# ak110/object_detector

Measured on AMD Instinct MI355X. Metric: images_per_sec, higher is better.
Workload: dtype f16

## Files before the change

### object_detector_amd/csrc/common.h

```cpp
#pragma once
#include <hip/hip_runtime.h>
#include <stdarg.h>
#include <stdint.h>
#include <stdio.h>
#include <string.h>

#include <unordered_map>

#include "../../include/odhip.h"

struct od_ctx {
  int device;
  void* zero_page;
  float* ones;
  int num_cu;
  std::unordered_map<const void*, size_t> lds_attr;
};

int od_ensure_lds(od_ctx* ctx, const void* fn, size_t lds);

void od_set_error(const char* fmt, ...);

#define OD_CHECK_HIP(expr)                                                                   \
  do {                                                                                       \
// ... 15 lines not shown

#define OD_REQUIRE(cond, ...)   \
  do {                          \
    if (!(cond)) {              \
      od_set_error(__VA_ARGS__); \
      return OD_ERR_INVALID;    \
    }                           \
  } while (0)

typedef _Float16 f16;
typedef f16 f16x8 __attribute__((ext_vector_type(8)));
typedef f16 f16x4 __attribute__((ext_vector_type(4)));
typedef float f32x4 __attribute__((ext_vector_type(4)));

static inline int od_ceil_div(int a, int b) { return (a + b - 1) / b; }
static inline int od_round_up(int a, int b) { return od_ceil_div(a, b) * b; }

struct od_launch {
  const char* name;
  int (*issue)(const od_launch& l, hipStream_t stream);
  const void* fn;
  dim3 grid, block;
  size_t lds;
  alignas(16) unsigned char args[352];
  template <class T> const T& arg() const { return *reinterpret_cast<const T*>(args); }
};
struct od_launches {
  int n = 0;
  od_launch l[6];
};

template <class T>
int od_add_launch(od_launches* L, od_launch l, const T& args) {
  static_assert(sizeof(T) <= sizeof(l.args) && alignof(T) <= 16, "kernel arguments do not fit an od_launch");
  OD_REQUIRE(L->n < 6, "%s: more than 6 launches in one op", l.name);
  memcpy(l.args, &args, sizeof(T));
  L->l[L->n++] = l;
  return OD_OK;
}
static inline int od_issue(const od_launches& L, hipStream_t stream) {
  for (int i = 0; i < L.n; ++i)
    if (int rc = L.l[i].issue(L.l[i], stream)) return rc;
  return OD_OK;
}

template <class F, class... A>
int od_prepare_issue(void* stream, F prepare, A... args) {
// ... 44 lines not shown
```

### object_detector_amd/csrc/conv_8ph_kernel.h

```cpp
#pragma once
#include "conv_8ph_tile.h"
#include "conv_common.h"

namespace {

constexpr int E_ALO = 0, E_AHI = E_REGION, E_BLO = 2 * E_REGION, E_BHI = 3 * E_REGION;

struct TapWalk {
  int c0, tap, tapoff, dx;
  int sel_tap;
};

constexpr unsigned E_OOB = 0x80000000u;

template <int MT, int NF = 4, bool KEEP = false>
static __device__ __forceinline__ void e8_epilogue_rt(const ConvKP& p, f32x4 (&acc)[MT][NF], int m0w, int n0w, int l15,
                                                          int lq, f16x8 (*keep)[NF / 2] = nullptr, int mrows = MT * 16,
                                                          const float* pre_sc = nullptr, const float* pre_bi = nullptr) {
  unsigned pb[MT], ppix[MT];
#pragma unroll
  for (int i = 0; i < MT; ++i) {
    const int m = m0w + i * 16 + l15;
    pb[i] = (unsigned)m / (unsigned)p.HoWo;
    ppix[i] = (unsigned)m - pb[i] * (unsigned)p.HoWo;
  }
#pragma unroll
  for (int pr = 0; pr < NF / 2; ++pr) {
    const int n = n0w + (2 * pr + (lq & 1)) * 16 + (lq >> 1) * 8;
    const bool nok = n < p.Cout;
    float sc[8], bi[8];
    if (pre_sc) {
#pragma unroll
      for (int e = 0; e < 8; ++e) {
        sc[e] = pre_sc[e];
        bi[e] = pre_bi[e];
      }
    } else {
      const f32x4 s0 = *(const f32x4*)(p.scale + n), s1 = *(const f32x4*)(p.scale + n + 4);
      const f32x4 b0 = *(const f32x4*)(p.bias + n), b1 = *(const f32x4*)(p.bias + n + 4);
#pragma unroll
      for (int e = 0; e < 4; ++e) {
        sc[e] = s0[e];
        sc[4 + e] = s1[e];
        bi[e] = b0[e];
        bi[4 + e] = b1[e];
      }
    }
    f16x8 rv[MT];
#pragma unroll
    for (int i = 0; i < MT; ++i) {
      const int m = m0w + i * 16 + l15;
      f16x8 r = {0, 0, 0, 0, 0, 0, 0, 0};
      if (nok && m < p.M && p.res_mode != OD_RES_NONE) {
        long long roff;
        if (p.res_mode == OD_RES_SAME) {
          roff = (long long)m * p.Cout + n;
        } else {
          const unsigned ho = ppix[i] / (unsigned)p.Wo, wo = ppix[i] - ho * (unsigned)p.Wo;
          roff = ((long long)(pb[i] * (unsigned)(p.Ho >> 1) + (ho >> 1)) * (p.Wo >> 1) + (wo >> 1)) * p.Cout + n;
        }
        r = *(const f16x8*)(p.res + roff);
      }
      rv[i] = r;
    }
#pragma unroll
    for (int i = 0; i < MT; ++i) {
      const int m = m0w + i * 16 + l15;
      const bool ok = nok && m < p.M && i * 16 + l15 < mrows;
      float v[8];
#pragma unroll
      for (int e = 0; e < 4; ++e) {
        float a = acc[i][2 * pr][e], bq = acc[i][2 * pr + 1][e];
        od_permlane16_swap(a, bq);
        v[e] = a;
        v[4 + e] = bq;
      }
#pragma unroll
      for (int e = 0; e < 8; ++e) v[e] = v[e] * sc[e] + bi[e];
      if (p.act == OD_ACT_LEAKY) {
#pragma unroll
        for (int e = 0; e < 8; ++e) v[e] = od_leaky(v[e], p.alpha);
      } else if (p.act == OD_ACT_ELU) {
#pragma unroll
        for (int e = 0; e < 8; ++e) v[e] = v[e] > 0.f ? v[e] : p.alpha * od_expm1_fast(v[e]);
      }
      if (p.res_mode != OD_RES_NONE) {
#pragma unroll
        for (int e = 0; e < 8; ++e) v[e] += (float)rv[i][e];
      }
      if (ok) {
        const long long ooff = (long long)pb[i] * p.obs + (long long)ppix[i] * p.ops + n;
        if (p.out_f32) {
          float* o = (float*)p.out + ooff;
          *(f32x4*)o = f32x4{v[0], v[1], v[2], v[3]};
          *(f32x4*)(o + 4) = f32x4{v[4], v[5], v[6], v[7]};
        } else {
          f16x8 h;
#pragma unroll
          for (int e = 0; e < 8; ++e) h[e] = (f16)v[e];
          *(f16x8*)((f16*)p.out + ooff) = h;
        }
      }
      if (KEEP) {
        f16x8 h;
#pragma unroll
        for (int e = 0; e < 8; ++e) h[e] = (f16)v[e];
        keep[i][pr] = h;
      }
    }
  }
}

template <int EPI, int MT, int NF, bool KEEP>
static __device__ __forceinline__ void e8_epilogue_fixed(const ConvKP& p, f32x4 (&acc)[MT][NF], int m0w, int n0w, int l15, int lq,
                                                         f16x8 (*keep)[NF / 2], int mrows, const float* pre_sc,
                                                         const float* pre_bi) {
  constexpr int ACT = od_epi_act(EPI), RES = od_epi_res(EPI);
  constexpr bool F32 = od_epi_f32(EPI);
  unsigned orow[MT], rrow[RES != OD_RES_NONE ? MT : 1];
#pragma unroll
  for (int i = 0; i < MT; ++i) {
    const unsigned m = (unsigned)min(m0w + i * 16 + l15, p.M - 1);
    const unsigned b = m / (unsigned)p.HoWo, pix = m - b * (unsigned)p.HoWo;
    orow[i] = b * (unsigned)p.obs + pix * (unsigned)p.ops;
    if (RES == OD_RES_SAME) rrow[i] = m * (unsigned)p.Cout;
    if (RES == OD_RES_UP2) {
      const unsigned ho = pix / (unsigned)p.Wo, wo = pix - ho * (unsigned)p.Wo;
      rrow[i] = ((b * (unsigned)(p.Ho >> 1) + (ho >> 1)) * (unsigned)(p.Wo >> 1) + (wo >> 1)) * (unsigned)p.Cout;
    }
  }
#pragma unroll
  for (int pr = 0; pr < NF / 2; ++pr) {
    const int n = n0w + (2 * pr + (lq & 1)) * 16 + (lq >> 1) * 8;
    const bool nok = n < p.Cout;
    float sc[8], bi[8];
    if (pre_sc) {
#pragma unroll
      for (int e = 0; e < 8; ++e) {
        sc[e] = pre_sc[e];
        bi[e] = pre_bi[e];
      }
    } else {
      const f32x4 s0 = *(const f32x4*)(p.scale + n), s1 = *(const f32x4*)(p.scale + n + 4);
      const f32x4 b0 = *(const f32x4*)(p.bias + n), b1 = *(const f32x4*)(p.bias + n + 4);
#pragma unroll
      for (int e = 0; e < 4; ++e) {
        sc[e] = s0[e];
        sc[4 + e] = s1[e];
        bi[e] = b0[e];
        bi[4 + e] = b1[e];
      }
// ... 49 lines not shown
  if constexpr (EPI == OD_EPI_RT)
    e8_epilogue_rt<MT, NF, KEEP>(p, acc, m0w, n0w, l15, lq, keep, mrows, pre_sc, pre_bi);
  else
    e8_epilogue_fixed<EPI, MT, NF, KEEP>(p, acc, m0w, n0w, l15, lq, keep, mrows, pre_sc, pre_bi);
}

template <int KS, int MF1, int EPI, int EPI2, bool PW, bool SEG>
__global__ __launch_bounds__(512, 2) void od_conv_8ph(ConvKP p_in) {
  constexpr int MF0 = 4, MT = MF0 + MF1, WROWS = MT * 16, BM = 2 * WROWS;
  extern __shared__ __attribute__((aligned(16))) char smem[];
  const int tid = threadIdx.x;
  const int lane = tid & 63;
  const int wave = __builtin_amdgcn_readfirstlane(tid >> 6);
  const int wr = wave >> 2, wc = wave & 3;
  const int l15 = lane & 15, lq = lane >> 4;

  int logical;
  {
    const int nt = p_in.mtiles * p_in.ntiles;
    const int pid = p_in.splitk > 1 ? (int)blockIdx.x / p_in.splitk : (int)blockIdx.x;
    const int q = nt >> 3, r = nt & 7, xcd = pid & 7, loc = pid >> 3;
    logical = (xcd < r ? xcd * (q + 1) : r * (q + 1) + (xcd - r) * q) + loc;
  }
  int tm = logical / p_in.ntiles;
  const int tn = logical - tm * p_in.ntiles;
  ConvKP p_seg;
  if (SEG) p_seg = p_in;
  if (SEG && p_in.nseg > 1) {
    int sg = 0;
    if (tm >= p_in.seg_tile0[1]) sg = 1;
    if (p_in.nseg > 2 && tm >= p_in.seg_tile0[2]) sg = 2;
    tm -= p_in.seg_tile0[sg];
    p_seg.x = p_in.seg_x[sg];
    p_seg.out = p_in.seg_out[sg];
    p_seg.H = p_seg.Ho = p_in.seg_H[sg];
    p_seg.W = p_seg.Wo = p_in.seg_W[sg];
    p_seg.HoWo = p_seg.H * p_seg.W;
    p_seg.M = p_in.seg_M[sg];
    p_seg.x_bytes = (unsigned)p_seg.M * (unsigned)p_in.Cin * 2u;
    if (p_in.obs == 0) p_seg.obs = (long long)p_seg.HoWo * p_in.Cout;
  }
  const ConvKP& p = SEG ? p_seg : p_in;
  const int m0 = tm * BM, n0 = tn * E_BN;
  const int nk_all = p.Ktot / E_BK;
  const int ks0 = p.splitk > 1 ? ((int)blockIdx.x % p.splitk) * p.steps_per_split : 0;
  const int nk = p.splitk > 1 ? min(p.steps_per_split, nk_all - ks0) : nk_all;
  if (nk <= 0) return;

  const int rr = tid >> 3;
  const int lc = (tid & 7) ^ (rr & 7);
  int a_base[2][2];
  unsigned a_vmask[2][2];
  unsigned a_sel[2][2];
#pragma unroll
  for (int s = 0; s < 2; ++s)
#pragma unroll
    for (int j = 0; j < 2; ++j) {
      const int m = m0 + j * WROWS + s * 64 + rr;
      a_vmask[s][j] = 0u;
      a_base[s][j] = 0;
      if (m < p.M && (s == 0 || rr < MF1 * 16)) {
        const unsigned b = (unsigned)m / (unsigned)p.HoWo;
        const unsigned pix = (unsigned)m - b * (unsigned)p.HoWo;
        const unsigned ho = pix / (unsigned)p.Wo;
        const unsigned wo = pix - ho * (unsigned)p.Wo;
        const int hi0 = (int)ho * p.stride - p.pad, wi0 = (int)wo * p.stride - p.pad;
        a_base[s][j] = ((((int)b * p.H + hi0 + p.pad) * p.W + wi0 + p.pad) * p.Cin + lc * 8) * 2;
#pragma unroll
        for (int t = 0; t < KS * KS; ++t) {
          const int hi = hi0 + t / KS, wi = wi0 + t % KS;
          if ((unsigned)hi < (unsigned)p.H && (unsigned)wi < (unsigned)p.W) a_vmask[s][j] |= 1u << t;
        }
      }
    }
  int w_off[2][2];
#pragma unroll
  for (int s = 0; s < 2; ++s)
#pragma unroll
    for (int j = 0; j < 2; ++j) {
      const int n = n0 + (2 * j + (rr >> 5)) * 64 + s * 32 + (rr & 31);
      w_off[s][j] = (n * p.Kstride + lc * 8 + ks0 * E_BK) * 2;
    }
  const __amdgpu_buffer_rsrc_t rs_x = __builtin_amdgcn_make_buffer_rsrc(
      (void*)(p.x - (long long)p.pad * (p.W + 1) * p.Cin), 0, (int)(p.x_bytes + (unsigned)(p.pad * (p.W + 1) * p.Cin * 2)),
      0x00020000);
  const __amdgpu_buffer_rsrc_t rs_w = __builtin_amdgcn_make_buffer_rsrc((void*)p.w, 0, (int)p.w_bytes, 0x00020000);
  auto blds16 = [&](const __amdgpu_buffer_rsrc_t& rs, unsigned voff, int soff, char* lptr) {
    __builtin_amdgcn_raw_ptr_buffer_load_lds(rs, (__attribute__((address_space(3))) void*)lptr, 16, (int)voff, soff, 0, 0);
  };

  auto walk_init = [&](TapWalk& w, int kt) {
    const int k0 = kt * E_BK;
    if (KS == 3) {
      w.sel_tap = -1;
      w.tap = k0 / p.Cin;
      w.c0 = k0 - w.tap * p.Cin;
      const int dy = w.tap / 3;
      w.dx = w.tap - dy * 3;
      w.tapoff = (dy * p.W + w.dx) * p.Cin;
    } else {
      w.sel_tap = -1;
      w.tap = 0;
      w.c0 = k0;
      w.dx = 0;
      w.tapoff = 0;
    }
  };
  auto walk_next = [&](TapWalk& w) {
    w.c0 += E_BK;
    if (KS == 3 && w.c0 >= p.Cin) {
      w.c0 = 0;
      ++w.tap;
      if (++w.dx == 3) {
        w.dx = 0;
        w.tapoff += (p.W - 2) * p.Cin;
      } else {
        w.tapoff += p.Cin;
      }
// ... 4 lines not shown
  walk_init(walk_hi, ks0);

  char* const piece = smem + wave * 1024;
  auto stage_a = [&](int s, TapWalk& w, int buf) {
    const int koff = w.tapoff + w.c0;
    char* dst = piece + buf * E_BUF + (s ? E_AHI : E_ALO);
    if (w.sel_tap != w.tap) {
      w.sel_tap = w.tap;
#pragma unroll
      for (int j = 0; j < 2; ++j) a_sel[s][j] = ((a_vmask[s][j] >> w.tap) & 1u) ? (unsigned)a_base[s][j] : E_OOB;
    }
#pragma unroll
    for (int j = 0; j < 2; ++j) blds16(rs_x, a_sel[s][j], koff * 2, dst + j * 8192);
    walk_next(w);
  };
  auto stage_b = [&](int s, int t, int buf) {
    char* dst = piece + buf * E_BUF + (s ? E_BHI : E_BLO);
#pragma unroll
    for (int j = 0; j < 2; ++j) blds16(rs_w, (unsigned)w_off[s][j], t * (E_BK * 2), dst + j * 8192);
  };

  const int w2buf = ((nk - 1) & 1) ^ 1;
  const __amdgpu_buffer_rsrc_t rs_w2 =
      __builtin_amdgcn_make_buffer_rsrc((void*)(PW ? p.w2 : p.w), 0, (int)(PW ? p.w2_bytes : p.w_bytes), 0x00020000);
  auto stage_w2 = [&](int ks) {
#pragma unroll
    for (int h = 0; h < 2; ++h)
      blds16(rs_w2, (unsigned)(((h * 64 + rr) * p.K2stride + lc * 8) * 2), ks * (E_BK * 2),
             piece + w2buf * E_BUF + ks * E_REGION + h * 8192);
  };

  f32x4 acc[MT][4];
#pragma unroll
  for (int i = 0; i < MT; ++i)
#pragma unroll
    for (int j = 0; j < 4; ++j) acc[i][j] = f32x4{0.f, 0.f, 0.f, 0.f};

  stage_a(0, walk_lo, 0);
  stage_b(0, 0, 0);
  stage_b(1, 0, 0);
  stage_a(1, walk_hi, 0);
  if (nk > 1) {
    stage_a(0, walk_lo, 1);
    stage_b(0, 1, 1);
    wait_vmcnt<8>();
  } else {
    wait_vmcnt<0>();
// ... 125 lines not shown
      const f32x4 b0 = *(const f32x4*)(p.bias2 + n2), b1 = *(const f32x4*)(p.bias2 + n2 + 4);
#pragma unroll
      for (int e = 0; e < 4; ++e) {
        sc2[e] = s0[e];
        sc2[4 + e] = s1[e];
        bi2[e] = b0[e];
        bi2[4 + e] = b1[e];
      }
    }
    f16x8 ykeep[MT][2];
    od_mfma_results_ready();
    e8_epilogue_direct<MT, 4, true, EPI>(p, acc, m0 + wr * WROWS, n0 + wc * 64, l15, lq, ykeep);
    ConvKP p2 = p;
    p2.scale = p.scale2;
    p2.bias = p.bias2;
    p2.act = p.act2;
    p2.alpha = p.alpha2;
    p2.res_mode = OD_RES_NONE;
    p2.out = (void*)p.out2;
    p2.out_f32 = 0;
    p2.Cout = p.Cout2;
    p2.obs = (long long)p.HoWo * p.Cout2;
    p2.ops = p.Cout2;
    char* const ybuf = smem + (w2buf ^ 1) * E_BUF;
    const char* const wbuf = smem + w2buf * E_BUF;
    const int fy = (rg * 64 + l15) * 128 + ((lq ^ (l15 & 7)) * 16);
    const int fw = (cg * 32 + l15) * 128 + ((lq ^ (l15 & 7)) * 16);
#pragma unroll
    for (int half = 0; half < 2; ++half) {
      if (wr == half) {
#pragma unroll
        for (int i = 0; i < MT; ++i)
#pragma unroll
          for (int pr = 0; pr < 2; ++pr) {
            const int row = i * 16 + l15;
            const int chunk = (2 * pr + (lq & 1)) * 2 + (lq >> 1);
            *(f16x8*)(ybuf + wc * E_REGION + row * 128 + ((chunk ^ (row & 7)) * 16)) = ykeep[i][pr];
          }
      }
      asm volatile("s_waitcnt lgkmcnt(0)" ::: "memory");
      __builtin_amdgcn_s_barrier();
      f32x4 acc2[4][2];
#pragma unroll
      for (int i = 0; i < 4; ++i)
#pragma unroll
        for (int f = 0; f < 2; ++f) acc2[i][f] = f32x4{0.f, 0.f, 0.f, 0.f};
// ... 31 lines not shown
```

### object_detector_amd/csrc/conv_common.h

```cpp
#pragma once
#include "common.h"

struct ConvKP {
  const f16* x;
  const f16* w;
  const float* scale;
  const float* bias;
  const f16* res;
  void* out;
  const f16* zero;
  int H, W, Cin, Ho, Wo, Cout;
  int stride, pad;
  int Kstride, Ktot, M, HoWo;
  int act;
  float alpha;
  int res_mode, out_f32;
  long long obs, ops;
  int mtiles, ntiles;
  int splitk, steps_per_split;
  float* ws;
  int Mq;
  int tconv, Hs, Ws;
  unsigned x_bytes, w_bytes;
  float* stats;
  const f16* w2;
  const float* scale2;
  const float* bias2;
  f16* out2;
  int Cout2, act2;
  float alpha2;
  unsigned w2_bytes;
  int K2stride;
  int nseg;
  int seg_tile0[4];
  const f16* seg_x[3];
  void* seg_out[3];
  int seg_H[3], seg_W[3], seg_M[3];
  int off32;
};

static __device__ __forceinline__ void glds16(const void* gptr, void* lptr) {
  __builtin_amdgcn_global_load_lds((const __attribute__((address_space(1))) void*)gptr,
                                   (__attribute__((address_space(3))) void*)lptr, 16, 0, 0);
}

static __device__ __forceinline__ float od_expm1_fast(float v) {
  const float poly = v * (1.f + v * (0.5f + v * (1.f / 6 + v * (1.f / 24 + v * (1.f / 120 + v * (1.f / 720))))));
  return v > -0.25f ? poly : __expf(v) - 1.f;
}

static __device__ __forceinline__ float od_elu_select(float v, float alpha) {
  const float poly = v * (1.f + v * (0.5f + v * (1.f / 6 + v * (1.f / 24 + v * (1.f / 120 + v * (1.f / 720))))));
  const float ex = __expf(v) - 1.f;
  const float em = v > -0.25f ? poly : ex;
  const float neg = alpha * em;
  return v > 0.f ? v : neg;
}

#define OD_EPI_RT -1
#define OD_EPI_LEAKY_NONE_F16 1
#define OD_EPI_LEAKY_SAME_F16 5
#define OD_EPI_ELU_NONE_F16 2
// ... 83 lines not shown
  }
  float st0[STATS ? 8 : 1], st1[STATS ? 8 : 1];
  if (STATS) {
#pragma unroll
    for (int e = 0; e < 8; ++e) st0[e] = st1[e] = 0.f;
  }
  constexpr int NPASS = (WTM + RPP - 1) / RPP;
  constexpr bool RAGGED = (WTM % RPP) != 0;
  f16x8 resv[WM][NPASS];
  if (res_mode != OD_RES_NONE && !splitk) {
#pragma unroll
    for (int wr = 0; wr < WM; ++wr)
#pragma unroll
      for (int ps = 0; ps < NPASS; ++ps) {
        int m = m0 + wr * WTM + ps * RPP + tid / CH;
        f16x8 r = {0, 0, 0, 0, 0, 0, 0, 0};
        if (RAGGED && ps * RPP + tid / CH >= WTM) m = p.M;
        if (tconv && m < p.M) m = od_tconv_pixel(p, (unsigned)m, WM * MT * 16);
        if (m >= 0 && m < p.M && n < p.Cout) {
          long long roff;
          if (res_mode == OD_RES_SAME) {
            roff = (long long)m * p.Cout + n;
          } else {
            const unsigned b = (unsigned)m / (unsigned)p.HoWo;
            const unsigned pix = (unsigned)m - b * (unsigned)p.HoWo;
            const unsigned ho = pix / (unsigned)p.Wo, wo = pix - ho * (unsigned)p.Wo;
            roff = ((long long)(b * (unsigned)(p.Ho >> 1) + (ho >> 1)) * (p.Wo >> 1) + (wo >> 1)) * p.Cout + n;
          }
          r = *(const f16x8*)(p.res + roff);
        }
        resv[wr][ps] = r;
      }
  }
#pragma unroll
  for (int wr = 0; wr < WM; ++wr) {
    if (wm == wr) {
#pragma unroll
      for (int j = 0; j < NTL; ++j) {
        const int nl = wn * WTN + j * 16 + lq * 4;
#pragma unroll
        for (int i = 0; i < MT; ++i) *(f32x4*)(stg + (i * 16 + l15) * SLD + nl) = acc[i][j];
      }
    }
    __syncthreads();
    if (splitk) {
      float* slab = p.ws + (long long)((int)blockIdx.x % p.splitk) * p.M * p.Cout;
#pragma unroll
      for (int ps = 0; ps < NPASS; ++ps) {
        const int row = ps * RPP + tid / CH;
// ... 12 lines not shown
      const int row = ps * RPP + tid / CH;
      int m = (RAGGED && row >= WTM) ? p.M : m0 + wr * WTM + row;
      if (tconv && m < p.M) m = od_tconv_pixel(p, (unsigned)m, WM * MT * 16);
      if (m >= 0 && m < p.M && n < p.Cout) {
        const f32x4 v0 = *(const f32x4*)(stg + row * SLD + c8);
        const f32x4 v1 = *(const f32x4*)(stg + row * SLD + c8 + 4);
        float v[8] = {v0[0], v0[1], v0[2], v0[3], v1[0], v1[1], v1[2], v1[3]};
        if (!STATS) {
#pragma unroll
          for (int e = 0; e < 8; ++e) v[e] = v[e] * sc[e] + bi[e];
        }
        if (STATS) {
        } else if (act == OD_ACT_LEAKY) {
#pragma unroll
          for (int e = 0; e < 8; ++e) v[e] = od_leaky(v[e], p.alpha);
        } else if (act == OD_ACT_ELU) {
#pragma unroll
          for (int e = 0; e < 8; ++e) v[e] = FX ? od_elu_select(v[e], p.alpha) : (v[e] > 0.f ? v[e] : p.alpha * od_expm1_fast(v[e]));
        }
        if (!STATS && res_mode != OD_RES_NONE) {
#pragma unroll
          for (int e = 0; e < 8; ++e) v[e] += (float)resv[wr][ps][e];
        }
        const unsigned b = (unsigned)m / (unsigned)p.HoWo;
        const unsigned pix = (unsigned)m - b * (unsigned)p.HoWo;
        const long long ooff = FX ? (long long)(b * (unsigned)p.obs + pix * (unsigned)p.ops + (unsigned)n)
                                  : (long long)b * p.obs + (long long)pix * p.ops + n;
        if (out_f32) {
          float* o = (float*)p.out + ooff;
          *(f32x4*)o = f32x4{v[0], v[1], v[2], v[3]};
          *(f32x4*)(o + 4) = f32x4{v[4], v[5], v[6], v[7]};
        } else {
          f16x8 h;
#pragma unroll
          for (int e = 0; e < 8; ++e) h[e] = (f16)v[e];
          *(f16x8*)((f16*)p.out + ooff) = h;
          if (STATS) {
#pragma unroll
            for (int e = 0; e < 8; ++e) {
              const float q = (float)h[e];
              st0[e] += q;
              st1[e] += q * q;
            }
          }
        }
      }
    }
    if (wr + 1 < WM) __syncthreads();
  }
  if (STATS) {
// ... 67 lines not shown
```

### object_detector_amd/csrc/conv_dispatch.hip

```cpp
#include <string.h>

#include "conv_common.h"

namespace {

int pick_cfg(const od_ctx* ctx, int M, int Cin, int Cout, int ksize, bool e8_ok, bool throughput) {
  const int cus = ctx->num_cu;
  const int cfg_e8 = od_conv_igemm_num_cfgs();
  const bool spec_ok = (Cin % 64) == 0;
  if (Cout <= 64) return (ksize == 3 && od_ceil_div(M, 128) >= 8 * cus) ? 1 : 3;
  const long t128 = (long)od_ceil_div(M, 128) * od_ceil_div(Cout, 128);
  if (ksize == 1) {
    if (!spec_ok) return 3;
    if (M <= 4096) return (M >= 2048 && Cin >= 512) ? 6 : 3;
    if (M <= 16384) return 7;
    if (Cout < 256) return 3;
    if (t128 < cus) return 4;
  }
  if (!spec_ok) return t128 >= 2L * cus ? 0 : 2;
  const int nk = od_ceil_div(ksize * ksize * Cin, 64);
  if (throughput && e8_ok && ksize == 3 && Cout >= 192 && M >= 2048) {
    double best = t128 >= cus ? t128 * (7.5 + 1.07 * nk) * 0.5 : t128 * (10.0 + 0.55 * nk);
    int pick = t128 >= cus ? 4 : (Cout <= 256 ? 7 : 5);
    for (int i = 0; i < od_conv_8ph_num_cfgs(); ++i) {
// ... 111 lines not shown
  p.Kstride = od_round_up(p.Ktot, 64);
  p.act = d->act;
  p.alpha = d->alpha;
  p.res_mode = d->res_mode;
  p.out_f32 = d->out_dtype == OD_DT_F32;
  p.stats = d->bn_partials;
  p.w2 = nullptr;
  p.scale2 = d->scale2;
  p.bias2 = d->bias2;
  p.out2 = (f16*)d->out2;
  p.Cout2 = d->Cout2;
  p.act2 = d->act2;
  p.alpha2 = d->alpha2;
  p.K2stride = od_round_up(d->Cout, 64);
  p.w2_bytes = (unsigned)((long long)od_round_up(d->Cout2 > 0 ? d->Cout2 : 1, 256) * p.K2stride * 2);
  p.x_bytes = (unsigned)((grouped ? seg_x_max : (long long)d->B * d->H * d->W * d->Cin) * 2);
  p.w_bytes = (unsigned)((long long)od_round_up(d->Cout, 256) * p.Kstride * 2);
  p.obs = d->out_batch_stride ? d->out_batch_stride : (long long)p.HoWo * d->Cout;
  p.ops = d->out_pix_stride ? d->out_pix_stride : d->Cout;
  long long hw_max = p.HoWo;
  for (int i = 0; grouped && i < d->nseg; ++i) hw_max = hw_max > (long long)d->seg_H[i] * d->seg_W[i] ? hw_max : (long long)d->seg_H[i] * d->seg_W[i];
  p.off32 = p.obs >= 0 && p.ops >= 0 && (long long)d->B * p.obs < (1LL << 31) &&
            (long long)(d->B - 1) * p.obs + (hw_max - 1) * p.ops + d->Cout < (1LL << 31);
  p.splitk = 1;
  p.steps_per_split = 0;
  p.ws = (float*)d->splitk_workspace;
  return OD_OK;
}

int conv_choose_cfg(const od_ctx* ctx, const od_conv_desc* d, const ConvKP& p, bool want_stats, int* cfg_out) {
  int cfg = d->tile_cfg;
  if (cfg < 0)
    cfg = pick_cfg(ctx, p.M, d->Cin, d->Cout, d->ksize, !want_stats && !p.tconv && (long long)p.x_bytes < 0x7F000000LL, cfg == -2);
  const int cfg_e8 = od_conv_igemm_num_cfgs();
  OD_REQUIRE(cfg < cfg_e8 + od_conv_8ph_num_cfgs(), "od_conv2d_fwd: tile_cfg %d out of range", cfg);
  OD_REQUIRE(!(want_stats && cfg >= cfg_e8), "od_conv2d_fwd: bn_partials is supported by the table kernels only (tile_cfg %d)", cfg);
  OD_REQUIRE(!p.tconv || cfg < cfg_e8, "od_conv2d_fwd: transposed mode runs on the table kernels only (tile_cfg %d)", cfg);
  *cfg_out = cfg;
  return OD_OK;
}

int conv_select(int cfg, const od_conv_desc* d, const ConvKP& p, bool want_stats, ConvKernelInfo* k) {
  const int cfg_e8 = od_conv_igemm_num_cfgs();
  if (cfg >= cfg_e8) {
    if (od_conv_8ph_select(cfg - cfg_e8, p, d->ksize, k)) return OD_OK;
    od_set_error("od_conv2d_fwd: tile_cfg %d (8-phase kernel) needs Cin %% 64 == 0 and no transposed gather", cfg);
    return OD_ERR_INVALID;
  }
  if (od_conv_igemm_select(cfg, d->ksize, d->Cin, want_stats, od_epi_of(p), k)) return OD_OK;
  od_set_error("od_conv2d_fwd: tile_cfg %d needs Cin %% %d == 0 for 3x3 (Cin = %d); use cfg 0-3", cfg, k->BK, d->Cin);
  return OD_ERR_INVALID;
}

void conv_tile_kp(const od_conv_desc* d, const ConvKernelInfo& k, ConvKP* kp) {
  ConvKP& p = *kp;
  p.mtiles = od_ceil_div(p.M, k.BM);
  if (p.nseg > 1) {
    int t0 = 0;
    for (int i = 0; i < 3; ++i) {
      const bool used = i < d->nseg;
      p.seg_tile0[i] = t0;
      p.seg_x[i] = used ? (const f16*)d->seg_x[i] : nullptr;
      p.seg_out[i] = used ? d->seg_out[i] : nullptr;
      p.seg_H[i] = used ? d->seg_H[i] : 0;
      p.seg_W[i] = used ? d->seg_W[i] : 0;
      p.seg_M[i] = d->B * p.seg_H[i] * p.seg_W[i];
      t0 += od_ceil_div(p.seg_M[i], k.BM);
    }
    p.seg_tile0[3] = t0;
    p.mtiles = t0;
    if (!d->out_batch_stride) p.obs = 0;
  }
  p.Mq = 0;
  if (p.tconv) {
    p.Mq = p.M / 4;
    p.mtiles = 4 * od_ceil_div(p.Mq, k.BM);
    p.M = p.mtiles * k.BM;
  }
  p.ntiles = od_ceil_div(d->Cout, k.BN);
}

int conv_prepare(od_ctx* ctx, const od_conv_desc* desc, bool want_stats, od_launches* L) {
  od_conv_desc v;
  ConvKP p;
  if (int rc = conv_describe(ctx, desc, want_stats, &v, &p)) return rc;
  const od_conv_desc* d = &v;
  const bool grouped = p.nseg > 1;
  if (d->tile_cfg < 0 && !want_stats && !grouped) {
    if (p.tconv && od_tconv_small_supported(d)) return od_tconv_small_prepare(ctx, d, L);
    if (od_conv_rdirect_supported(d)) return od_conv_rdirect_prepare(ctx, d, L);
    if (!p.tconv && od_conv_stream3_supported(d)) return od_conv_stream3_prepare(ctx, d, L);
  }
  int cfg;
  if (int rc = conv_choose_cfg(ctx, d, p, want_stats, &cfg)) return rc;
  const bool use_e8 = cfg >= od_conv_igemm_num_cfgs();
  if (grouped && !(use_e8 && d->Cin % 64 == 0)) {
    od_conv_desc q = *d;
    q.nseg = 0;
    for (int i = 0; i < d->nseg; ++i) {
      q.x = d->seg_x[i];
      q.out = d->seg_out[i];
      q.H = d->seg_H[i];
// ... 122 lines not shown
```

### object_detector_amd/csrc/conv_mfma.hip

```cpp
#include <stdlib.h>
#include <string.h>

#include "conv_common.h"

namespace {

template <int BM, int BN, int BK, int STAGES, int WM, int WN, int SPEC = 0>
struct ConvCfg {
  static constexpr int NT = WM * WN * 64;
  static constexpr int NTHREADS = NT * (SPEC ? 2 : 1);
  static constexpr int CPR = BK / 8;
  static constexpr int RPR = NT / CPR;
  static constexpr int AR = BM / RPR, BR = BN / RPR;
  static constexpr int ROWB = BK * 2;
  static constexpr int A_BYTES = BM * ROWB, B_BYTES = BN * ROWB, STAGE_BYTES = A_BYTES + B_BYTES;
  static constexpr int WTM = BM / WM, WTN = BN / WN;
  static constexpr int MT = WTM / 16, NTL = WTN / 16;
  static constexpr int SLD = BN + 4;
  static constexpr int PIPE_BYTES = STAGES * STAGE_BYTES;
  static constexpr int EPI_BYTES = WTM * SLD * 4;
  static constexpr int LDS_BYTES = PIPE_BYTES > EPI_BYTES ? PIPE_BYTES : EPI_BYTES;
  static constexpr int LOADS = AR + BR;
  static_assert(BM % RPR == 0 && BN % RPR == 0, "tile must be a whole number of DMA rounds");
  static_assert(BK == 32 || BK == 64, "BK");
// ... 5 lines not shown
__global__ __launch_bounds__(WM* WN * 64 * (SPEC ? 2 : 1), MINW) void od_conv_igemm(ConvKP p) {
  using Cf = ConvCfg<BM, BN, BK, STAGES, WM, WN, SPEC>;
  constexpr int NT = Cf::NT, AR = Cf::AR, BR = Cf::BR, RPR = Cf::RPR, ROWB = Cf::ROWB;
  constexpr int WTM = Cf::WTM, WTN = Cf::WTN, MT = Cf::MT, NTL = Cf::NTL;

  extern __shared__ __attribute__((aligned(16))) char smem[];

  const int tid_all = threadIdx.x;
  const int lane = tid_all & 63;
  const int wave_all = __builtin_amdgcn_readfirstlane(tid_all >> 6);
  const bool is_loader = SPEC ? (wave_all >= WM * WN) : true;
  const bool is_consumer = SPEC ? (wave_all < WM * WN) : true;
  const int tid = SPEC ? (tid_all & (NT - 1)) : tid_all;
  const int wave = SPEC ? (wave_all >= WM * WN ? wave_all - WM * WN : wave_all) : wave_all;
  const int l15 = lane & 15, lq = lane >> 4;

  int logical;
  {
    const int nt = p.mtiles * p.ntiles;
    const int pid = p.splitk > 1 ? (int)blockIdx.x / p.splitk : (int)blockIdx.x;
    const int q = nt >> 3, r = nt & 7, xcd = pid & 7, loc = pid >> 3;
    logical = (xcd < r ? xcd * (q + 1) : r * (q + 1) + (xcd - r) * q) + loc;
  }
  const int tm = logical / p.ntiles, tn = logical - tm * p.ntiles;
  const int m0 = tm * BM, n0 = tn * BN;
  const int nk_all = (p.Ktot + BK - 1) / BK;
  const int ks0 = p.splitk > 1 ? ((int)blockIdx.x % p.splitk) * p.steps_per_split : 0;
  int nk = p.splitk > 1 ? min(p.steps_per_split, nk_all - ks0) : nk_all;
  if (nk <= 0) return;

  int rr, lc, piece_off;
  if (BK == 64) {
    rr = tid >> 3;
    lc = (tid & 7) ^ (rr & 7);
    piece_off = wave * 8 * ROWB;
  } else {
    rr = wave * 16 + (lane & 15);
    lc = lane >> 4;
    piece_off = wave * 16 * ROWB;
  }
  int a_base[AR], a_hi0[AR], a_wi0[AR], a_b[AR];
  unsigned a_vmask[AR];
#pragma unroll
  for (int rd = 0; rd < AR; ++rd) {
    int m = m0 + rd * RPR + rr;
    a_vmask[rd] = 0u;
    if (p.tconv && m < p.M) m = od_tconv_pixel(p, (unsigned)m, BM);
    if (m >= 0 && m < p.M) {
      const unsigned b = (unsigned)m / (unsigned)p.HoWo;
      const unsigned pix = (unsigned)m - b * (unsigned)p.HoWo;
      const unsigned ho = pix / (unsigned)p.Wo;
      const unsigned wo = pix - ho * (unsigned)p.Wo;
      a_hi0[rd] = (int)ho * p.stride - p.pad;
      a_wi0[rd] = (int)wo * p.stride - p.pad;
      a_base[rd] = (((int)b * p.H + a_hi0[rd]) * p.W + a_wi0[rd]) * p.Cin + lc * 8;
      a_b[rd] = (int)b;
#pragma unroll
      for (int t = 0; t < KS * KS; ++t) {
        const int hi = a_hi0[rd] + t / KS, wi = a_wi0[rd] + t % KS;
        bool ok = (unsigned)hi < (unsigned)p.H && (unsigned)wi < (unsigned)p.W;
        if (p.tconv) ok = ok && !((hi | wi) & 1);
        if (ok) a_vmask[rd] |= 1u << t;
      }
    } else {
      a_hi0[rd] = -(1 << 24);
      a_wi0[rd] = 0;
      a_base[rd] = 0;
      a_b[rd] = 0;
    }
  }
  const f16* wrow = p.w + (long long)(n0 + rr) * p.Kstride + lc * 8;

  unsigned tmask = 0x1FFu;
  if (UNI && KS == 3 && p.tconv && p.splitk <= 1) {
    unsigned um = 0u;
#pragma unroll
    for (int rd = 0; rd < AR; ++rd) um |= a_vmask[rd];
    for (int off = 32; off; off >>= 1) um |= (unsigned)__shfl_xor((int)um, off, 64);
    unsigned* sh = (unsigned*)smem;
    if (tid_all == 0) *sh = 0u;
    __syncthreads();
    if (lane == 0) atomicOr(sh, um);
    __syncthreads();
    tmask = (unsigned)__builtin_amdgcn_readfirstlane((int)*sh);
    __syncthreads();
    nk = __builtin_popcount(tmask) * (p.Cin / BK);
  }

  int ld_k0 = ks0 * BK, ld_c0 = ld_k0, ld_tap = 0, ld_tapoff = 0, ld_dx = 0, ld_dy = 0;
  if (UNI && KS == 3) {
    ld_tap = ld_k0 / p.Cin;
    ld_c0 = ld_k0 - ld_tap * p.Cin;
    if (tmask != 0x1FFu && tmask != 0u) {
      ld_tap = __builtin_ctz(tmask);
      ld_c0 = 0;
      ld_k0 = ld_tap * p.Cin;
    }
    ld_dy = ld_tap / 3;
    ld_dx = ld_tap - ld_dy * 3;
    ld_tapoff = (ld_dy * p.W + ld_dx) * p.Cin;
  }

  constexpr int NX = AR + BR;
  f16x8 rtmp[SPEC == 2 ? NX : 1];
  char* rdst[SPEC == 2 ? NX : 1];
  int rn = 0;
  auto xfer = [&](const f16* src, char* lds_piece) {
    if (SPEC == 2) {
      rtmp[rn] = *(const f16x8*)src;
      rdst[rn] = lds_piece + lane * 16;
      ++rn;
    } else {
      glds16(src, lds_piece);
    }
  };
  auto stage = [&](int buf) {
    rn = 0;
    char* abuf = smem + buf * Cf::STAGE_BYTES + piece_off;
    char* bbuf = abuf + Cf::A_BYTES;
    if (UNI) {
      const bool cvalid = (KS == 3) || (ld_c0 + lc * 8 < p.Cin);
      const int koff = ld_tapoff + ld_c0;
#pragma unroll
      for (int rd = 0; rd < AR; ++rd) {
        const bool ok = cvalid && ((a_vmask[rd] >> ld_tap) & 1u);
        const f16* src;
        if (KS == 3 && p.tconv) {
          const int u = (a_hi0[rd] + ld_dy) >> 1, v = (a_wi0[rd] + ld_dx) >> 1;
          src = ok ? p.x + (((a_b[rd] * p.Hs + u) * p.Ws + v) * p.Cin + lc * 8 + ld_c0) : p.zero;
        } else {
          src = ok ? p.x + (a_base[rd] + koff) : p.zero;
        }
        xfer(src, abuf + rd * RPR * ROWB);
      }
    } else {
      const int k = ld_k0 + lc * 8;
      const int tap = k / p.Cin;
      const int dy = tap / 3, dx = tap - dy * 3;
      const int cin = k - tap * p.Cin;
      const bool kvalid = k < p.Ktot;
      const int koff = (dy * p.W + dx) * p.Cin + cin - lc * 8;
#pragma unroll
      for (int rd = 0; rd < AR; ++rd) {
        const int hi = a_hi0[rd] + dy, wi = a_wi0[rd] + dx;
        const bool ok = kvalid && (unsigned)hi < (unsigned)p.H && (unsigned)wi < (unsigned)p.W;
        const f16* src = ok ? p.x + (a_base[rd] + koff) : p.zero;
        xfer(src, abuf + rd * RPR * ROWB);
      }
    }
#pragma unroll
    for (int rd = 0; rd < BR; ++rd) xfer(wrow + (long long)rd * RPR * p.Kstride + ld_k0, bbuf + rd * RPR * ROWB);
    if (SPEC == 2) {
#pragma unroll
      for (int i = 0; i < NX; ++i) *(f16x8*)rdst[i] = rtmp[i];
    }
    ld_k0 += BK;
    if (UNI) {
      ld_c0 += BK;
      if (KS == 3 && ld_c0 >= p.Cin) {
        ld_c0 = 0;
// ... 83 lines not shown

__global__ __launch_bounds__(256) void od_conv_finish(ConvKP p) {
  const long long nvec = (long long)p.M * (p.Cout >> 3);
  const int C8 = p.Cout >> 3;
  for (long long i = (long long)blockIdx.x * 256 + threadIdx.x; i < nvec; i += (long long)gridDim.x * 256) {
    const int m = (int)(i / C8), n = (int)(i - (long long)m * C8) * 8;
    const float* wsp = p.ws + (long long)m * p.Cout + n;
    const long long slab = (long long)p.M * p.Cout;
    float v[8] = {0.f, 0.f, 0.f, 0.f, 0.f, 0.f, 0.f, 0.f};
    for (int sidx = 0; sidx < p.splitk; ++sidx) {
      const f32x4 a0 = *(const f32x4*)(wsp + sidx * slab), a1 = *(const f32x4*)(wsp + sidx * slab + 4);
#pragma unroll
      for (int e = 0; e < 4; ++e) {
        v[e] += a0[e];
        v[4 + e] += a1[e];
      }
    }
#pragma unroll
    for (int e = 0; e < 8; ++e) {
      v[e] = v[e] * p.scale[n + e] + p.bias[n + e];
      if (p.act == OD_ACT_LEAKY) v[e] = od_leaky(v[e], p.alpha);
      else if (p.act == OD_ACT_ELU) v[e] = v[e] > 0.f ? v[e] : p.alpha * od_expm1_fast(v[e]);
    }
    const unsigned b = (unsigned)m / (unsigned)p.HoWo;
    const unsigned pix = (unsigned)m - b * (unsigned)p.HoWo;
    if (p.res_mode != OD_RES_NONE) {
      long long roff;
      if (p.res_mode == OD_RES_SAME) {
        roff = (long long)m * p.Cout + n;
      } else {
        const unsigned ho = pix / (unsigned)p.Wo, wo = pix - ho * (unsigned)p.Wo;
        roff = ((long long)(b * (unsigned)(p.Ho >> 1) + (ho >> 1)) * (p.Wo >> 1) + (wo >> 1)) * p.Cout + n;
      }
      const f16x8 r = *(const f16x8*)(p.res + roff);
#pragma unroll
      for (int e = 0; e < 8; ++e) v[e] += (float)r[e];
    }
    const long long ooff = (long long)b * p.obs + (long long)pix * p.ops + n;
    if (p.out_f32) {
      float* o = (float*)p.out + ooff;
      *(f32x4*)o = f32x4{v[0], v[1], v[2], v[3]};
      *(f32x4*)(o + 4) = f32x4{v[4], v[5], v[6], v[7]};
    } else {
      f16x8 h;
#pragma unroll
      for (int e = 0; e < 8; ++e) h[e] = (f16)v[e];
      *(f16x8*)((f16*)p.out + ooff) = h;
    }
  }
}

struct TileCfg {
  int BM, BN, BK, threads;
  size_t lds;
// ... 62 lines not shown
```

Baseline: 22780.

## Replace runtime integer divisions with precomputed fastdiv and add dense/identity index fast paths

Precomputes magic-multiplier divisors for HoWo, Wo, Cin and ntiles on the host and uses them in the conv kernels instead of hardware-less 32-bit integer division. Adds a dense-output flag so epilogues compute offsets as m*Cout without splitting the row index, and an identity flag so 1x1 stride-1 convs skip pixel decomposition and tap masks entirely. Tap masks are built as row*column bitmasks, and buffer resource pointers and offsets are forced scalar via readfirstlane. The kernel argument block grows, and the launch-args buffer is enlarged to fit, which adds parameter size and some risk if a fastdiv encoding is wrong for edge divisors.

```diff
diff --git a/object_detector_amd/csrc/common.h b/object_detector_amd/csrc/common.h
--- a/object_detector_amd/csrc/common.h
+++ b/object_detector_amd/csrc/common.h
@@ -61,7 +61,7 @@
   const void* fn;
   dim3 grid, block;
   size_t lds;
-  alignas(16) unsigned char args[352];
+  alignas(16) unsigned char args[480];
   template <class T> const T& arg() const { return *reinterpret_cast<const T*>(args); }
 };
 struct od_launches {
diff --git a/object_detector_amd/csrc/conv_8ph_kernel.h b/object_detector_amd/csrc/conv_8ph_kernel.h
--- a/object_detector_amd/csrc/conv_8ph_kernel.h
+++ b/object_detector_amd/csrc/conv_8ph_kernel.h
@@ -17,12 +17,12 @@
 static __device__ __forceinline__ void e8_epilogue_rt(const ConvKP& p, f32x4 (&acc)[MT][NF], int m0w, int n0w, int l15,
                                                           int lq, f16x8 (*keep)[NF / 2] = nullptr, int mrows = MT * 16,
                                                           const float* pre_sc = nullptr, const float* pre_bi = nullptr) {
+  const bool flat = p.dense && p.res_mode != OD_RES_UP2;
   unsigned pb[MT], ppix[MT];
 #pragma unroll
   for (int i = 0; i < MT; ++i) {
-    const int m = m0w + i * 16 + l15;
-    pb[i] = (unsigned)m / (unsigned)p.HoWo;
-    ppix[i] = (unsigned)m - pb[i] * (unsigned)p.HoWo;
+    pb[i] = ppix[i] = 0u;
+    if (!flat) od_row_split(p, (unsigned)(m0w + i * 16 + l15), pb[i], ppix[i]);
   }
 #pragma unroll
   for (int pr = 0; pr < NF / 2; ++pr) {
@@ -56,7 +56,8 @@
         if (p.res_mode == OD_RES_SAME) {
           roff = (long long)m * p.Cout + n;
         } else {
-          const unsigned ho = ppix[i] / (unsigned)p.Wo, wo = ppix[i] - ho * (unsigned)p.Wo;
+          unsigned ho, wo;
+          od_pix_split(p, ppix[i], ho, wo);
           roff = ((long long)(pb[i] * (unsigned)(p.Ho >> 1) + (ho >> 1)) * (p.Wo >> 1) + (wo >> 1)) * p.Cout + n;
         }
         r = *(const f16x8*)(p.res + roff);
@@ -89,7 +90,7 @@
         for (int e = 0; e < 8; ++e) v[e] += (float)rv[i][e];
       }
       if (ok) {
-        const long long ooff = (long long)pb[i] * p.obs + (long long)ppix[i] * p.ops + n;
+        const long long ooff = p.dense ? (long long)m * p.Cout + n : (long long)pb[i] * p.obs + (long long)ppix[i] * p.ops + n;
         if (p.out_f32) {
           float* o = (float*)p.out + ooff;
           *(f32x4*)o = f32x4{v[0], v[1], v[2], v[3]};
@@ -118,15 +119,26 @@
   constexpr int ACT = od_epi_act(EPI), RES = od_epi_res(EPI);
   constexpr bool F32 = od_epi_f32(EPI);
   unsigned orow[MT], rrow[RES != OD_RES_NONE ? MT : 1];
-#pragma unroll
-  for (int i = 0; i < MT; ++i) {
-    const unsigned m = (unsigned)min(m0w + i * 16 + l15, p.M - 1);
-    const unsigned b = m / (unsigned)p.HoWo, pix = m - b * (unsigned)p.HoWo;
-    orow[i] = b * (unsigned)p.obs + pix * (unsigned)p.ops;
-    if (RES == OD_RES_SAME) rrow[i] = m * (unsigned)p.Cout;
-    if (RES == OD_RES_UP2) {
-      const unsigned ho = pix / (unsigned)p.Wo, wo = pix - ho * (unsigned)p.Wo;
-      rrow[i] = ((b * (unsigned)(p.Ho >> 1) + (ho >> 1)) * (unsigned)(p.Wo >> 1) + (wo >> 1)) * (unsigned)p.Cout;
+  if (p.dense && RES != OD_RES_UP2) {
+#pragma unroll
+    for (int i = 0; i < MT; ++i) {
+      const unsigned m = (unsigned)min(m0w + i * 16 + l15, p.M - 1);
+      orow[i] = m * (unsigned)p.Cout;
+      if (RES == OD_RES_SAME) rrow[i] = orow[i];
+    }
+  } else {
+#pragma unroll
+    for (int i = 0; i < MT; ++i) {
+      const unsigned m = (unsigned)min(m0w + i * 16 + l15, p.M - 1);
+      unsigned b, pix;
+      od_row_split(p, m, b, pix);
+      orow[i] = b * (unsigned)p.obs + pix * (unsigned)p.ops;
+      if (RES == OD_RES_SAME) rrow[i] = m * (unsigned)p.Cout;
+      if (RES == OD_RES_UP2) {
+        unsigned ho, wo;
+        od_pix_split(p, pix, ho, wo);
+        rrow[i] = ((b * (unsigned)(p.Ho >> 1) + (ho >> 1)) * (unsigned)(p.Wo >> 1) + (wo >> 1)) * (unsigned)p.Cout;
+      }
     }
   }
 #pragma unroll
@@ -222,7 +234,7 @@
     const int q = nt >> 3, r = nt & 7, xcd = pid & 7, loc = pid >> 3;
     logical = (xcd < r ? xcd * (q + 1) : r * (q + 1) + (xcd - r) * q) + loc;
   }
-  int tm = logical / p_in.ntiles;
+  int tm = od_fastdiv_uniform(logical, p_in.d_ntiles);
   const int tn = logical - tm * p_in.ntiles;
   ConvKP p_seg;
   if (SEG) p_seg = p_in;
@@ -236,6 +248,8 @@
     p_seg.H = p_seg.Ho = p_in.seg_H[sg];
     p_seg.W = p_seg.Wo = p_in.seg_W[sg];
     p_seg.HoWo = p_seg.H * p_seg.W;
+    p_seg.d_howo = p_in.seg_d_howo[sg];
+    p_seg.d_wo = p_in.seg_d_wo[sg];
     p_seg.M = p_in.seg_M[sg];
     p_seg.x_bytes = (unsigned)p_seg.M * (unsigned)p_in.Cin * 2u;
     if (p_in.obs == 0) p_seg.obs = (long long)p_seg.HoWo * p_in.Cout;
@@ -260,16 +274,16 @@
       a_vmask[s][j] = 0u;
       a_base[s][j] = 0;
       if (m < p.M && (s == 0 || rr < MF1 * 16)) {
-        const unsigned b = (unsigned)m / (unsigned)p.HoWo;
-        const unsigned pix = (unsigned)m - b * (unsigned)p.HoWo;
-        const unsigned ho = pix / (unsigned)p.Wo;
-        const unsigned wo = pix - ho * (unsigned)p.Wo;
-        const int hi0 = (int)ho * p.stride - p.pad, wi0 = (int)wo * p.stride - p.pad;
-        a_base[s][j] = ((((int)b * p.H + hi0 + p.pad) * p.W + wi0 + p.pad) * p.Cin + lc * 8) * 2;
-#pragma unroll
-        for (int t = 0; t < KS * KS; ++t) {
-          const int hi = hi0 + t / KS, wi = wi0 + t % KS;
-          if ((unsigned)hi < (unsigned)p.H && (unsigned)wi < (unsigned)p.W) a_vmask[s][j] |= 1u << t;
+        if (KS == 1 && p.ident) {
+          a_base[s][j] = (m * p.Cin + lc * 8) * 2;
+          a_vmask[s][j] = 1u;
+        } else {
+          unsigned b, pix, ho, wo;
+          od_row_split(p, (unsigned)m, b, pix);
+          od_pix_split(p, pix, ho, wo);
+          const int hi0 = (int)ho * p.stride - p.pad, wi0 = (int)wo * p.stride - p.pad;
+          a_base[s][j] = ((((int)b * p.H + hi0 + p.pad) * p.W + wi0 + p.pad) * p.Cin + lc * 8) * 2;
+          a_vmask[s][j] = od_tap_mask<KS>(hi0, wi0, p.H, p.W);
         }
       }
     }
@@ -281,19 +295,26 @@
       const int n = n0 + (2 * j + (rr >> 5)) * 64 + s * 32 + (rr & 31);
       w_off[s][j] = (n * p.Kstride + lc * 8 + ks0 * E_BK) * 2;
     }
+  auto uni_ptr = [](const void* q) {
+    const unsigned long long a = (unsigned long long)q;
+    const unsigned lo = (unsigned)__builtin_amdgcn_readfirstlane((int)(unsigned)a);
+    const unsigned hi = (unsigned)__builtin_amdgcn_readfirstlane((int)(unsigned)(a >> 32));
+    return (void*)(((unsigned long long)hi << 32) | lo);
+  };
   const __amdgpu_buffer_rsrc_t rs_x = __builtin_amdgcn_make_buffer_rsrc(
-      (void*)(p.x - (long long)p.pad * (p.W + 1) * p.Cin), 0, (int)(p.x_bytes + (unsigned)(p.pad * (p.W + 1) * p.Cin * 2)),
-      0x00020000);
-  const __amdgpu_buffer_rsrc_t rs_w = __builtin_amdgcn_make_buffer_rsrc((void*)p.w, 0, (int)p.w_bytes, 0x00020000);
+      uni_ptr(p.x - (long long)p.pad * (p.W + 1) * p.Cin), 0,
+      __builtin_amdgcn_readfirstlane((int)(p.x_bytes + (unsigned)(p.pad * (p.W + 1) * p.Cin * 2))), 0x00020000);
+  const __amdgpu_buffer_rsrc_t rs_w = __builtin_amdgcn_make_buffer_rsrc(uni_ptr(p.w), 0, (int)p.w_bytes, 0x00020000);
   auto blds16 = [&](const __amdgpu_buffer_rsrc_t& rs, unsigned voff, int soff, char* lptr) {
-    __builtin_amdgcn_raw_ptr_buffer_load_lds(rs, (__attribute__((address_space(3))) void*)lptr, 16, (int)voff, soff, 0, 0);
+    __builtin_amdgcn_raw_ptr_buffer_load_lds(rs, (__attribute__((address_space(3))) void*)lptr, 16, (int)voff,
+                                             __builtin_amdgcn_readfirstlane(soff), 0, 0);
   };
 
   auto walk_init = [&](TapWalk& w, int kt) {
     const int k0 = kt * E_BK;
     if (KS == 3) {
       w.sel_tap = -1;
-      w.tap = k0 / p.Cin;
+      w.tap = od_fastdiv_uniform(k0, p.d_cin);
       w.c0 = k0 - w.tap * p.Cin;
       const int dy = w.tap / 3;
       w.dx = w.tap - dy * 3;
@@ -344,7 +365,7 @@
 
   const int w2buf = ((nk - 1) & 1) ^ 1;
   const __amdgpu_buffer_rsrc_t rs_w2 =
-      __builtin_amdgcn_make_buffer_rsrc((void*)(PW ? p.w2 : p.w), 0, (int)(PW ? p.w2_bytes : p.w_bytes), 0x00020000);
+      __builtin_amdgcn_make_buffer_rsrc(uni_ptr(PW ? p.w2 : p.w), 0, (int)(PW ? p.w2_bytes : p.w_bytes), 0x00020000);
   auto stage_w2 = [&](int ks) {
 #pragma unroll
     for (int h = 0; h < 2; ++h)
@@ -516,6 +537,7 @@
     p2.Cout = p.Cout2;
     p2.obs = (long long)p.HoWo * p.Cout2;
     p2.ops = p.Cout2;
+    p2.dense = 1;
     char* const ybuf = smem + (w2buf ^ 1) * E_BUF;
     const char* const wbuf = smem + w2buf * E_BUF;
     const int fy = (rg * 64 + l15) * 128 + ((lq ^ (l15 & 7)) * 16);
diff --git a/object_detector_amd/csrc/conv_common.h b/object_detector_amd/csrc/conv_common.h
--- a/object_detector_amd/csrc/conv_common.h
+++ b/object_detector_amd/csrc/conv_common.h
@@ -1,5 +1,6 @@
 #pragma once
 #include "common.h"
+#include "fastdiv.h"
 
 struct ConvKP {
   const f16* x;
@@ -37,7 +38,35 @@
   void* seg_out[3];
   int seg_H[3], seg_W[3], seg_M[3];
   int off32;
+  od_fastdiv d_howo, d_wo, d_cin, d_ntiles;
+  od_fastdiv seg_d_howo[3], seg_d_wo[3];
+  int dense;
+  int ident;
 };
+
+static __device__ __forceinline__ void od_row_split(const ConvKP& p, unsigned m, unsigned& b, unsigned& pix) {
+  b = od_fastdiv_div(m, p.d_howo);
+  pix = m - b * (unsigned)p.HoWo;
+}
+static __device__ __forceinline__ void od_pix_split(const ConvKP& p, unsigned pix, unsigned& ho, unsigned& wo) {
+  ho = od_fastdiv_div(pix, p.d_wo);
+  wo = pix - ho * (unsigned)p.Wo;
+}
+static __device__ __forceinline__ int od_fastdiv_uniform(int n, const od_fastdiv& f) {
+  return __builtin_amdgcn_readfirstlane((int)od_fastdiv_div((unsigned)n, f));
+}
+template <int KS, bool EVEN = false>
+static __device__ __forceinline__ unsigned od_tap_mask(int hi0, int wi0, int H, int W) {
+  unsigned rows = 0u, cols = 0u;
+#pragma unroll
+  for (int d = 0; d < KS; ++d) {
+    const bool r = (unsigned)(hi0 + d) < (unsigned)H && !(EVEN && ((hi0 + d) & 1));
+    const bool c = (unsigned)(wi0 + d) < (unsigned)W && !(EVEN && ((wi0 + d) & 1));
+    rows |= r ? 1u << (d * KS) : 0u;
+    cols |= c ? 1u << d : 0u;
+  }
+  return rows * cols;
+}
 
 static __device__ __forceinline__ void glds16(const void* gptr, void* lptr) {
   __builtin_amdgcn_global_load_lds((const __attribute__((address_space(1))) void*)gptr,
@@ -167,9 +196,9 @@
           if (res_mode == OD_RES_SAME) {
             roff = (long long)m * p.Cout + n;
           } else {
-            const unsigned b = (unsigned)m / (unsigned)p.HoWo;
-            const unsigned pix = (unsigned)m - b * (unsigned)p.HoWo;
-            const unsigned ho = pix / (unsigned)p.Wo, wo = pix - ho * (unsigned)p.Wo;
+            unsigned b, pix, ho, wo;
+            od_row_split(p, (unsigned)m, b, pix);
+            od_pix_split(p, pix, ho, wo);
             roff = ((long long)(b * (unsigned)(p.Ho >> 1) + (ho >> 1)) * (p.Wo >> 1) + (wo >> 1)) * p.Cout + n;
           }
           r = *(const f16x8*)(p.res + roff);
@@ -228,10 +257,15 @@
 #pragma unroll
           for (int e = 0; e < 8; ++e) v[e] += (float)resv[wr][ps][e];
         }
-        const unsigned b = (unsigned)m / (unsigned)p.HoWo;
-        const unsigned pix = (unsigned)m - b * (unsigned)p.HoWo;
-        const long long ooff = FX ? (long long)(b * (unsigned)p.obs + pix * (unsigned)p.ops + (unsigned)n)
-                                  : (long long)b * p.obs + (long long)pix * p.ops + n;
+        long long ooff;
+        if (p.dense) {
+          ooff = FX ? (long long)((unsigned)m * (unsigned)p.Cout + (unsigned)n) : (long long)m * p.Cout + n;
+        } else {
+          unsigned b, pix;
+          od_row_split(p, (unsigned)m, b, pix);
+          ooff = FX ? (long long)(b * (unsigned)p.obs + pix * (unsigned)p.ops + (unsigned)n)
+                    : (long long)b * p.obs + (long long)pix * p.ops + n;
+        }
         if (out_f32) {
           float* o = (float*)p.out + ooff;
           *(f32x4*)o = f32x4{v[0], v[1], v[2], v[3]};
diff --git a/object_detector_amd/csrc/conv_dispatch.hip b/object_detector_amd/csrc/conv_dispatch.hip
--- a/object_detector_amd/csrc/conv_dispatch.hip
+++ b/object_detector_amd/csrc/conv_dispatch.hip
@@ -157,6 +157,13 @@
   for (int i = 0; grouped && i < d->nseg; ++i) hw_max = hw_max > (long long)d->seg_H[i] * d->seg_W[i] ? hw_max : (long long)d->seg_H[i] * d->seg_W[i];
   p.off32 = p.obs >= 0 && p.ops >= 0 && (long long)d->B * p.obs < (1LL << 31) &&
             (long long)(d->B - 1) * p.obs + (hw_max - 1) * p.ops + d->Cout < (1LL << 31);
+  p.d_howo = od_fastdiv_make((unsigned)p.HoWo);
+  p.d_wo = od_fastdiv_make((unsigned)p.Wo);
+  p.d_cin = od_fastdiv_make((unsigned)p.Cin);
+  p.d_ntiles = od_fastdiv_make(1u);
+  for (int i = 0; i < 3; ++i) p.seg_d_howo[i] = p.seg_d_wo[i] = od_fastdiv_make(1u);
+  p.dense = p.ops == d->Cout && (grouped ? d->out_batch_stride == 0 : p.obs == (long long)p.HoWo * p.ops);
+  p.ident = d->ksize == 1 && p.stride == 1 && !p.tconv;
   p.splitk = 1;
   p.steps_per_split = 0;
   p.ws = (float*)d->splitk_workspace;
@@ -200,6 +207,8 @@
       p.seg_H[i] = used ? d->seg_H[i] : 0;
       p.seg_W[i] = used ? d->seg_W[i] : 0;
       p.seg_M[i] = d->B * p.seg_H[i] * p.seg_W[i];
+      p.seg_d_howo[i] = od_fastdiv_make((unsigned)(p.seg_H[i] * p.seg_W[i]));
+      p.seg_d_wo[i] = od_fastdiv_make((unsigned)p.seg_W[i]);
       t0 += od_ceil_div(p.seg_M[i], k.BM);
     }
     p.seg_tile0[3] = t0;
@@ -213,6 +222,7 @@
     p.M = p.mtiles * k.BM;
   }
   p.ntiles = od_ceil_div(d->Cout, k.BN);
+  p.d_ntiles = od_fastdiv_make((unsigned)p.ntiles);
 }
 
 int conv_prepare(od_ctx* ctx, const od_conv_desc* desc, bool want_stats, od_launches* L) {
diff --git a/object_detector_amd/csrc/conv_mfma.hip b/object_detector_amd/csrc/conv_mfma.hip
--- a/object_detector_amd/csrc/conv_mfma.hip
+++ b/object_detector_amd/csrc/conv_mfma.hip
@@ -51,7 +51,7 @@
     const int q = nt >> 3, r = nt & 7, xcd = pid & 7, loc = pid >> 3;
     logical = (xcd < r ? xcd * (q + 1) : r * (q + 1) + (xcd - r) * q) + loc;
   }
-  const int tm = logical / p.ntiles, tn = logical - tm * p.ntiles;
+  const int tm = od_fastdiv_uniform(logical, p.d_ntiles), tn = logical - tm * p.ntiles;
   const int m0 = tm * BM, n0 = tn * BN;
   const int nk_all = (p.Ktot + BK - 1) / BK;
   const int ks0 = p.splitk > 1 ? ((int)blockIdx.x % p.splitk) * p.steps_per_split : 0;
@@ -76,20 +76,20 @@
     a_vmask[rd] = 0u;
     if (p.tconv && m < p.M) m = od_tconv_pixel(p, (unsigned)m, BM);
     if (m >= 0 && m < p.M) {
-      const unsigned b = (unsigned)m / (unsigned)p.HoWo;
-      const unsigned pix = (unsigned)m - b * (unsigned)p.HoWo;
-      const unsigned ho = pix / (unsigned)p.Wo;
-      const unsigned wo = pix - ho * (unsigned)p.Wo;
-      a_hi0[rd] = (int)ho * p.stride - p.pad;
-      a_wi0[rd] = (int)wo * p.stride - p.pad;
-      a_base[rd] = (((int)b * p.H + a_hi0[rd]) * p.W + a_wi0[rd]) * p.Cin + lc * 8;
-      a_b[rd] = (int)b;
-#pragma unroll
-      for (int t = 0; t < KS * KS; ++t) {
-        const int hi = a_hi0[rd] + t / KS, wi = a_wi0[rd] + t % KS;
-        bool ok = (unsigned)hi < (unsigned)p.H && (unsigned)wi < (unsigned)p.W;
-        if (p.tconv) ok = ok && !((hi | wi) & 1);
-        if (ok) a_vmask[rd] |= 1u << t;
+      if (KS == 1 && p.ident) {
+        a_hi0[rd] = a_wi0[rd] = a_b[rd] = 0;
+        a_base[rd] = m * p.Cin + lc * 8;
+        a_vmask[rd] = 1u;
+      } else {
+        unsigned b, pix, ho, wo;
+        od_row_split(p, (unsigned)m, b, pix);
+        od_pix_split(p, pix, ho, wo);
+        a_hi0[rd] = (int)ho * p.stride - p.pad;
+        a_wi0[rd] = (int)wo * p.stride - p.pad;
+        a_base[rd] = (((int)b * p.H + a_hi0[rd]) * p.W + a_wi0[rd]) * p.Cin + lc * 8;
+        a_b[rd] = (int)b;
+        a_vmask[rd] = p.tconv ? od_tap_mask<KS, true>(a_hi0[rd], a_wi0[rd], p.H, p.W)
+                              : od_tap_mask<KS, false>(a_hi0[rd], a_wi0[rd], p.H, p.W);
       }
     } else {
       a_hi0[rd] = -(1 << 24);
@@ -118,7 +118,7 @@
 
   int ld_k0 = ks0 * BK, ld_c0 = ld_k0, ld_tap = 0, ld_tapoff = 0, ld_dx = 0, ld_dy = 0;
   if (UNI && KS == 3) {
-    ld_tap = ld_k0 / p.Cin;
+    ld_tap = od_fastdiv_uniform(ld_k0, p.d_cin);
     ld_c0 = ld_k0 - ld_tap * p.Cin;
     if (tmask != 0x1FFu && tmask != 0u) {
       ld_tap = __builtin_ctz(tmask);
@@ -164,7 +164,7 @@
       }
     } else {
       const int k = ld_k0 + lc * 8;
-      const int tap = k / p.Cin;
+      const int tap = (int)od_fastdiv_div((unsigned)k, p.d_cin);
       const int dy = tap / 3, dx = tap - dy * 3;
       const int cin = k - tap * p.Cin;
       const bool kvalid = k < p.Ktot;
@@ -294,14 +294,15 @@
       if (p.act == OD_ACT_LEAKY) v[e] = od_leaky(v[e], p.alpha);
       else if (p.act == OD_ACT_ELU) v[e] = v[e] > 0.f ? v[e] : p.alpha * od_expm1_fast(v[e]);
     }
-    const unsigned b = (unsigned)m / (unsigned)p.HoWo;
-    const unsigned pix = (unsigned)m - b * (unsigned)p.HoWo;
+    unsigned b, pix;
+    od_row_split(p, (unsigned)m, b, pix);
     if (p.res_mode != OD_RES_NONE) {
       long long roff;
       if (p.res_mode == OD_RES_SAME) {
         roff = (long long)m * p.Cout + n;
       } else {
-        const unsigned ho = pix / (unsigned)p.Wo, wo = pix - ho * (unsigned)p.Wo;
+        unsigned ho, wo;
+        od_pix_split(p, pix, ho, wo);
         roff = ((long long)(b * (unsigned)(p.Ho >> 1) + (ho >> 1)) * (p.Wo >> 1) + (wo >> 1)) * p.Cout + n;
       }
       const f16x8 r = *(const f16x8*)(p.res + roff);
diff --git a/object_detector_amd/csrc/fastdiv.h b/object_detector_amd/csrc/fastdiv.h
--- /dev/null
+++ b/object_detector_amd/csrc/fastdiv.h
@@ -0,0 +1,27 @@
+#pragma once
+
+#if defined(__HIPCC__) || defined(__CUDACC__)
+#define OD_FASTDIV_FN __host__ __device__ __forceinline__
+#else
+#define OD_FASTDIV_FN inline
+#endif
+
+struct od_fastdiv {
+  unsigned mul, add, shift;
+};
+
+static inline od_fastdiv od_fastdiv_make(unsigned d) {
+  od_fastdiv f = {0xFFFFFFFFu, 0xFFFFFFFFu, 0u};
+  if (d <= 1u) return f;
+  unsigned l = 0;
+  while (l < 32 && (1ull << l) < d) ++l;
+  const unsigned long long two = 1ull << (31 + l);
+  f.mul = (unsigned)((two + d - 1) / d);
+  f.add = 0u;
+  f.shift = l - 1;
+  return f;
+}
+
+static OD_FASTDIV_FN unsigned od_fastdiv_div(unsigned n, const od_fastdiv& f) {
+  return (unsigned)(((unsigned long long)n * f.mul + f.add) >> 32) >> f.shift;
+}
```

After: 23050, median of 3. +1.2%, better.
